# real-space/tfQMRgpu

Hardware: AMD Instinct MI355X
Metric: tfQMR solve throughput to 1e-9 residual (reference flop count / solve time); iterations/s and BSR multiply GB/s + TFLOP/s in extra keys (higher is better)
Workload: dtype f64; 1 GPU; generate_FD_example 16 120 4 2 -0.25 n 0 4 (16x16 complex<double>); mb=3573, nnzbA=17589, nnzbX_per_gpu=138229, block_columns_per_gpu=49, rhs_per_gpu=784, pairs=679189

## Files before the change

### tfqmrgpu_amd/csrc/tfq_api.hip

```cpp
#include <cstdio>
#include <cstdlib>
#include <cstring>
#include <cmath>
#include <algorithm>
#include <new>
#include <vector>
#include <dlfcn.h>

#include "tfq_device.hpp"
#include "tfq_order.hpp"
#include "tfq_vec.hpp"
#include "tfq_switch.hpp"

using namespace tfq;

namespace tfq {

static inline char lower(char c) { return char(c | 32); }

DevPlan resolve(Plan const& p) {
    DevPlan d{};
    char* b = p.buffer;
    auto at = [&](Window const& w) { return (void*)(b + w.offset); };
    d.LM = p.LM; d.LN = p.LN; d.dbl = ('z' == p.precision);
// ... 218 lines not shown
                (void)hipHostFree(p.ring); p.ring = nullptr;
                return TFQ_ERR(TFQMRGPU_STATUS_ALLOCATION_FAILED);
            }
            e = (void*)ev_;
        }
    }
    Ctl* const ring = (Ctl*)p.ring;
    hipEvent_t ev[DEPTH];
    for (int i = 0; i < DEPTH; ++i) ev[i] = (hipEvent_t)p.ringEvent[i];
    int const prof = p.profiling;
    auto const timed = [prof](int k) { return 1 == prof || (2 == prof && (TFQMRGPU_PROF_SPMM_V4_DOT == k || TFQMRGPU_PROF_SPMM_V5_NRM_DOT == k)); };
    EventList pev;
    if (prof && !pev.create(size_t(DEPTH) * (NK + 1))) return TFQ_ERR(TFQMRGPU_STATUS_ALLOCATION_FAILED);

    { RoctxRange const range(roctx(), "tfQMR preparation"); TFQ_HIP(vec_launch(VEC_SETUP, d, tol, maxIt, s), TFQMRGPU_STATUS_LAUNCH_FAILED) }
    RoctxRange const range(roctx(), "tfQMR iterations");

    tfqmrgpuStatus_t fail = TFQMRGPU_STATUS_SUCCESS;

    auto const userOp = (tfqmrgpuOperator_t)p.opFn;
    double userFlops = 0;
    size_t const vecBytes = size_t(p.nnzbX) * 2 * p.LM * p.LN * (d.dbl ? 8 : 4);
    auto const up256 = [](size_t n) { return (n + 255) & ~size_t(255); };
    if (userOp && !p.opScratch) {
        size_t const bytes = 2 * up256(vecBytes) + up256(size_t(p.nnzbX) * 4) + up256(size_t(p.nnzbX) * 2);
        TFQ_HIP(hipMalloc((void**)&p.opScratch, bytes ? bytes : 256), TFQMRGPU_STATUS_ALLOCATION_FAILED)
        char* const q = p.opScratch + 2 * up256(vecBytes);
        std::vector<uint16_t> cu(p.nnzbX);
        for (uint32_t u = 0; u < p.nnzbX; ++u) cu[u] = p.colindx[u];
        TFQ_HIP(hipMemcpyAsync(q, p.i2u.data(), size_t(p.nnzbX) * 4, hipMemcpyHostToDevice, s), TFQMRGPU_STATUS_LAUNCH_FAILED)
        TFQ_HIP(hipMemcpyAsync(q + up256(size_t(p.nnzbX) * 4), cu.data(), size_t(p.nnzbX) * 2, hipMemcpyHostToDevice, s), TFQMRGPU_STATUS_LAUNCH_FAILED)
        TFQ_HIP(hipStreamSynchronize(s), TFQMRGPU_STATUS_LAUNCH_FAILED)
    }
    auto multiply = [&](int epi, DevPlan const& d) {
        if (!userOp) { spmm_launch(epi, d, s); return; }
        char* const xu = p.opScratch; char* const yu = xu + up256(vecBytes);
        auto const i2u = (uint32_t const*)(yu + up256(vecBytes));
        auto const colU = (uint16_t const*)((char const*)i2u + up256(size_t(p.nnzbX) * 4));
        launch_convert(1, d.dbl, d.dbl, (EPI_RESIDUAL == epi) ? d.x : d.v6, xu, d.u2i, 0, p.nnzbX, p.LM, p.LN,
                       TFQMRGPU_LAYOUT_RRRRIIII, false, false, p.ilv, s);
        double fl = 0;
        auto const st = userOp(p.opCtx, yu, xu, colU, p.nnzbX, p.nCols, p.LM, p.LN, p.precision, (tfqmrgpuStream_t)s, &fl);
        if (st && !fail) fail = st;
        userFlops += fl;
        epilogue_launch(epi, d, yu, i2u, s);
    };

    static double const kOne = 1.;
    auto reduce = [&](int what) {
        if (fail && hipSuccess != hipMemcpyAsync(&d.ctl->red[3 * what + 2], &kOne, sizeof kOne, hipMemcpyHostToDevice, s)) return;
        auto const st = reduce_over_ranks(h, &d.ctl->red[3 * what], 3, s);
        if (st && !fail) fail = st;
    };
    auto launches = [&](int slot, int part, bool firstIteration) {
        DevPlan const dSlot = [&] { DevPlan x = d; x.first = firstIteration ? 1 : 0; return x; }();
        auto mark = [&](int k) {
            if (!(k < NK && timed(k)) && !(k > 0 && timed(k - 1))) return;
            if (hipSuccess != hipEventRecord(pev[slot * (NK + 1) + k], s) && !fail) fail = TFQ_ERR(TFQMRGPU_STATUS_LAUNCH_FAILED);
        };
        if (part != 2) {
            mark(TFQMRGPU_PROF_DEC35);            (void)vec_launch(VEC_DEC35, d, 0, 0, s);
            mark(TFQMRGPU_PROF_XPAY_V6);          (void)vec_launch(VEC_XPAY_V6, dSlot, 0, 0, s);
            mark(TFQMRGPU_PROF_SPMM_V4_DOT);      multiply(EPI_XPAY_DOT, dSlot);
            mark(TFQMRGPU_PROF_DEC34);            if (!fold) (void)vec_launch(VEC_DEC34, d, 0, 0, s);
            mark(TFQMRGPU_PROF_V5_NRM);           (void)vec_launch(VEC_V5_NRM, dSlot, 0, 0, s);
            mark(TFQMRGPU_PROF_DECT_C67);         if (!fold) (void)vec_launch(VEC_DECT_C67, d, 0, 0, s);
            mark(TFQMRGPU_PROF_X_V6_V7);          (void)vec_launch(VEC_X_V6_V7, dSlot, 0, 0, s);
            mark(TFQMRGPU_PROF_SPMM_V5_NRM_DOT);  multiply(EPI_AXPY_NRM_DOT, dSlot);
            mark(TFQMRGPU_PROF_DECT_FINAL);       if (!fold) (void)vec_launch(VEC_DECT_FIN, d, 0, 0, s);
            mark(TFQMRGPU_PROF_DECIDE);
            if (multi) {
                launch_decide(d, 1, s);
                reduce(0);
                launch_decide(d, 2, s);
            } else if (!fold) launch_decide(d, 0, s);
            mark(TFQMRGPU_PROF_PROBE);
        }
        if (part != 1) {
            (void)vec_launch(VEC_X_FLUSH, d, 0, 0, s);
            multiply(EPI_RESIDUAL, dSlot);
            if (!fold) (void)vec_launch(VEC_PROBE_COL, d, 0, 0, s);
            if (multi) {
                launch_probe_decide(d, 1, s);
                reduce(1);
                launch_probe_decide(d, 2, s);
            } else if (!fold) launch_probe_decide(d, 0, s);
        }
        mark(NK);
    };
    auto enqueue = [&](int slot, int part, bool firstIteration) {
        launches(slot, part, firstIteration);
        if ((hipSuccess != hipMemcpyAsync(&ring[slot], d.ctl, sizeof(Ctl), hipMemcpyDeviceToHost, s) ||
             hipSuccess != hipEventRecord(ev[slot], s)) && !fail) fail = TFQ_ERR(TFQMRGPU_STATUS_LAUNCH_FAILED);
    };

    Ctl last{};
    last.state = (maxIt > 0) ? 0 : 3; last.residual2_reached = 1e300; last.iterations_needed = maxIt;
    int enq = 0, seen = 0;
    if (userOp) {
        for (int it = 0; it < maxIt && !fail && 0 == last.state; ++it) {
            for (int part = 1; part <= 2 && !fail; ++part) {
                if (2 == part && !(0 == last.state && last.probe)) break;
                enqueue(0, part, 0 == it);
                if (hipSuccess != hipEventSynchronize(ev[0])) { fail = TFQ_ERR(TFQMRGPU_STATUS_LAUNCH_FAILED); break; }
                last = ring[0];
                if (1 == part) p.boundHistory.push_back(last.max_bound2 * histScale);
            }
            if (prof) for (int k = 0; k < NK; ++k) {
                float ms = 0;
                if (timed(k) && hipSuccess == hipEventElapsedTime(&ms, pev[k], pev[k + 1])) {
                    p.profMs[k] += ms; p.profLaunches[k] += 1;
                    if (0 == it) { p.profFirstMs[k] += ms; p.profFirstLaunches[k] += 1; }
                }
            }
        }
    } else
    while (enq < std::min(ahead, maxIt)) { enqueue(enq % DEPTH, 0, 0 == enq); ++enq; }
    while (seen < enq && (!fail || multi)) {
        int const slot = seen % DEPTH;
        if (hipSuccess != hipEventSynchronize(ev[slot])) { if (!fail) fail = TFQ_ERR(TFQMRGPU_STATUS_LAUNCH_FAILED); break; }
        int const nprobes_before = last.nprobes;
        last = ring[slot];
        ++seen;
        p.boundHistory.push_back(last.max_bound2 * histScale);
        if (prof) for (int k = 0; k < NK; ++k) {
            if (!timed(k)) continue;
            bool const gated = (TFQMRGPU_PROF_PROBE == k && last.nprobes == nprobes_before);
            float ms = 0;
            if (hipSuccess == hipEventElapsedTime(&ms, pev[slot * (NK + 1) + k], pev[slot * (NK + 1) + k + 1])) {
                if (gated) { p.profGatedMs[k] += ms; p.profGatedLaunches[k] += 1; }
                else {
                    p.profMs[k] += ms; p.profLaunches[k] += 1;
                    if (1 == seen) { p.profFirstMs[k] += ms; p.profFirstLaunches[k] += 1; }
                }
            }
        }
        if (last.state != 0) break;
        if (enq < maxIt) { enqueue(enq % DEPTH, 0, false); ++enq; }
    }
// ... 731 lines not shown
```

### tfqmrgpu_amd/csrc/tfq_colops.hpp

```cpp
#pragma once
#include "tfq_device.hpp"

namespace tfq {

#define TFQ_EPS 2.5e-308

struct ColScratch { double s[512]; double rec[2][64]; double s0[256], s1[256]; int last; };

__device__ inline void co_store(double* p, double v) { double const old = __hip_atomic_exchange(p, v, __ATOMIC_RELAXED, __HIP_MEMORY_SCOPE_AGENT); asm volatile("" :: "v"(old)); }
__device__ inline double co_load(double const* p) { return __hip_atomic_load(p, __ATOMIC_RELAXED, __HIP_MEMORY_SCOPE_AGENT); }
__device__ inline void st_record(double* p, double v, bool coherent) { if (coherent) co_store(p, v); else *p = v; }

template <int LN, int NPL, bool COH = false>
__device__ inline void column_sum(double const* part, uint32_t c0, uint32_t c1, double* s, double (&res)[NPL]) {
    constexpr int G = 256 / LN;
    constexpr int U = 16;
    int const t = threadIdx.x, g = t / LN, j = t % LN;
    double acc[NPL] = {};
    if (g < G) {
        for (uint32_t c = c0 + g; c < c1; c += U * G) {
            double v[U][NPL];
#pragma unroll
            for (int u = 0; u < U; ++u)
#pragma unroll
                for (int p = 0; p < NPL; ++p) v[u][p] = (c + u * G < c1) ? (COH ? co_load(part + (size_t(c + u * G) * NPL + p) * LN + j) : part[(size_t(c + u * G) * NPL + p) * LN + j]) : 0.;
#pragma unroll
            for (int u = 0; u < U; ++u)
                if (c + u * G < c1)
#pragma unroll
                    for (int p = 0; p < NPL; ++p) acc[p] += v[u][p];
        }
    }
    __syncthreads();
    if (g < G)
#pragma unroll
        for (int p = 0; p < NPL; ++p) s[(g * NPL + p) * LN + j] = acc[p];
    __syncthreads();
#pragma unroll
    for (int p = 0; p < NPL; ++p) res[p] = 0;
    if (t < LN) for (int gg = 0; gg < G; ++gg)
#pragma unroll
        for (int p = 0; p < NPL; ++p) res[p] += s[(gg * NPL + p) * LN + t];
}

__device__ inline bool fold_arrive(uint32_t* counter, uint32_t expected, int* lastFlag) {
    asm volatile("s_waitcnt vmcnt(0)" ::: "memory");
    __syncthreads();
    if (0 == threadIdx.x) {
        uint32_t const before = __hip_atomic_fetch_add(counter, 1u, __ATOMIC_RELAXED, __HIP_MEMORY_SCOPE_AGENT);
        int const last = (before + 1 == expected) ? 1 : 0;
        if (last) __hip_atomic_store(counter, 0u, __ATOMIC_RELAXED, __HIP_MEMORY_SCOPE_AGENT);
        *lastFlag = last;
    }
    __syncthreads();
    return *lastFlag != 0;
}

__device__ inline size_t col_part_slot(uint32_t c0, uint32_t col, uint32_t seg) { return size_t(c0 / kColSlot) + col + seg; }

template <int LN, int NPL>
__device__ inline bool column_total(DevPlan const& d, double const* part, uint32_t col, int seg, double* s, int* lastFlag, double (&res)[NPL]) {
    uint32_t const c0 = d.colChunkPtr[col], c1 = d.colChunkPtr[col + 1], n = c1 - c0;
    uint32_t const S = (seg < 0) ? 1u : col_segments(n, LN);
    if (uint32_t(seg < 0 ? 0 : seg) >= S) return false;
    if (1 == S) { if (seg < 0) column_sum<LN, NPL, true>(part, c0, c1, s, res); else column_sum<LN, NPL>(part, c0, c1, s, res); return true; }
    uint32_t const len = (n + S - 1) / S, b0 = c0 + uint32_t(seg) * len, b1 = min(c1, b0 + len);
    column_sum<LN, NPL>(part, b0, b1, s, res);
    int const t = threadIdx.x;
    if (t < LN)
#pragma unroll
        for (int p = 0; p < NPL; ++p) co_store(d.colPart + (col_part_slot(c0, col, uint32_t(seg)) * 3 + p) * LN + t, res[p]);
    if (t < 64) asm volatile("s_waitcnt vmcnt(0)" ::: "memory");
    if (0 == t) {
        uint32_t const before = __hip_atomic_fetch_add(d.foldCount + col, 1u, __ATOMIC_RELAXED, __HIP_MEMORY_SCOPE_AGENT);
        int const last = (before + 1 == S) ? 1 : 0;
        if (last) __hip_atomic_store(d.foldCount + col, 0u, __ATOMIC_RELAXED, __HIP_MEMORY_SCOPE_AGENT);
        *lastFlag = last;
    }
    __syncthreads();
    if (0 == *lastFlag) return false;
    if (t < LN) {
#pragma unroll
        for (int p = 0; p < NPL; ++p) res[p] = 0;
        constexpr int U = 8;
        for (uint32_t g0 = 0; g0 < S; g0 += U) {
            double v[U][NPL];
#pragma unroll
            for (int u = 0; u < U; ++u)
#pragma unroll
                for (int p = 0; p < NPL; ++p)
                    v[u][p] = (g0 + u < S) ? co_load(d.colPart + (col_part_slot(c0, col, g0 + u) * 3 + p) * LN + t) : 0.;
#pragma unroll
            for (int u = 0; u < U; ++u)
                if (g0 + u < S)
#pragma unroll
                    for (int p = 0; p < NPL; ++p) res[p] += v[u][p];
        }
    }
    return true;
}

template <typename R, int LN>
__device__ inline void col_dec35(DevPlan const& d, uint32_t const col, double* s, int seg, int* lastFlag) {
    int const j = threadIdx.x, jc = (j < LN) ? j : LN - 1;
    size_t const ir = (size_t(col) * 2 + 0) * LN + jc, ii = ir + LN;
    R* rho = (R*)d.rho; R* bet = (R*)d.beta;
    double const rr = double(rho[ir]), ri = double(rho[ii]);
    double z[2];
    if (!column_total<LN, 2>(d, d.pz, col, seg, s, lastFlag, z)) return;
    if (j >= LN) return;
    double const abs2rho = rr * rr + ri * ri, abs2z = z[0] * z[0] + z[1] * z[1];
    d.z[ir] = z[0]; d.z[ii] = z[1];
    if (abs2z < TFQ_EPS || abs2rho < TFQ_EPS) {
        d.status[size_t(col) * LN + j] = -1;
        bet[ir] = 0; bet[ii] = 0; rho[ir] = 0; rho[ii] = 0;
    } else {
        double const den = 1. / abs2rho;
        bet[ir] = R((z[0] * rr + z[1] * ri) * den);
        bet[ii] = R((z[1] * rr - z[0] * ri) * den);
        rho[ir] = R(z[0]); rho[ii] = R(z[1]);
    }
}

template <typename R, int LN>
__device__ inline void col_dec34(DevPlan const& d, uint32_t const col, double* s, int seg, int* lastFlag) {
    int const j = threadIdx.x, jc = (j < LN) ? j : LN - 1;
    size_t const ir = (size_t(col) * 2 + 0) * LN + jc, ii = ir + LN;
    R const* rho = (R const*)d.rho; R const* eta = (R const*)d.eta2; R* alf = (R*)d.alfa; R* c67 = (R*)d.c67a;
    double const rr = double(rho[ir]), ri = double(rho[ii]);
    double const er = double(eta[ir]), ei = double(eta[ii]), var0 = d.var[size_t(col) * LN + jc];
    double z[2];
    if (!column_total<LN, 2>(d, d.pz, col, seg, s, lastFlag, z)) return;
    if (j >= LN) return;
    double const abs2rho = rr * rr + ri * ri, abs2z = z[0] * z[0] + z[1] * z[1];
    d.z[ir] = z[0]; d.z[ii] = z[1];
    if (abs2z < TFQ_EPS || abs2rho < TFQ_EPS) {
        d.status[size_t(col) * LN + j] = -2;
        alf[ir] = 0; alf[ii] = 0; c67[ir] = 0; c67[ii] = 0;
    } else {
        double const zden = -1. / abs2z;
        alf[ir] = R((rr * z[0] + ri * z[1]) * zden);
        alf[ii] = R((ri * z[0] - rr * z[1]) * zden);
        double const vden = var0 / abs2rho;
        double const tr = (er * rr + ei * ri) * vden, ti = (ei * rr - er * ri) * vden;
        c67[ir] = R(z[0] * tr - z[1] * ti);
        c67[ii] = R(z[1] * tr + z[0] * ti);
    }
}

template <typename R, int LN, bool SETC67, bool FINAL>
__device__ inline void col_decT(DevPlan const& d, uint32_t const col, double* s, double (*rec)[64], int seg, int* lastFlag) {
    int const j = threadIdx.x, jc = (j < LN) ? j : LN - 1;
    double const Tau0 = d.tau[size_t(col) * LN + jc];
    int8_t const st0 = d.status[size_t(col) * LN + jc];
    R const alr0 = ((R const*)d.alfa)[(size_t(col) * 2 + 0) * LN + jc], ali0 = ((R const*)d.alfa)[(size_t(col) * 2 + 1) * LN + jc];
    double const invB0 = FINAL ? d.invBn2[size_t(col) * LN + jc] : 0.;
    double dd[1];
    if (!column_total<LN, 1>(d, d.pd, col, seg, s, lastFlag, dd)) return;
    if (j < LN) {
        size_t const ir = (size_t(col) * 2 + 0) * LN + j, ii = ir + LN, i1 = size_t(col) * LN + j;
        R* eta = (R*)(FINAL ? d.eta2 : d.eta); R* c67 = (R*)d.c67;
        double cosi = 0; R r67 = 1;
        double const Tau = Tau0;
        int8_t st = st0;
        double newTau;
        if (fabs(Tau) > TFQ_EPS) {
            double const Var = dd[0] / Tau;
            cosi = 1. / (1. + Var);
            d.var[i1] = Var;
            newTau = dd[0] * cosi;
            r67 = R(Var * cosi);
        } else {
            st = -3; d.status[i1] = -3;
            d.var[i1] = 0; newTau = 0;
        }
        d.tau[i1] = newTau;
        d.d[i1] = dd[0];
        if (st < 0) { eta[ir] = 0; eta[ii] = 0; }
        else { eta[ir] = R(-cosi * alr0); eta[ii] = R(-cosi * ali0); }
        if (SETC67) { c67[ir] = r67; c67[ii] = 0; }
        if (FINAL) { rec[0][j] = newTau * invB0; rec[1][j] = (st == -1 || st == -2) ? 0. : 1.; }
    }
    if (FINAL) {
        __syncthreads();
        if (0 == j) {
            double mx = 0, alive = 0;
            for (int jj = 0; jj < LN; ++jj) { if (rec[0][jj] > mx) mx = rec[0][jj]; if (rec[1][jj] > alive) alive = rec[1][jj]; }
            st_record(d.colrec + size_t(col) * 2 + 0, mx, seg < 0); st_record(d.colrec + size_t(col) * 2 + 1, alive, seg < 0);
        }
    }
}

template <int LN>
__device__ inline void col_probe(DevPlan const& d, uint32_t const col, double* s, double (*rec)[64], int seg, int* lastFlag) {
    double dd[1];
    if (!column_total<LN, 1>(d, d.pd, col, seg, s, lastFlag, dd)) return;
    int const j = threadIdx.x;
    if (j < LN) {
        size_t const i1 = size_t(col) * LN + j;
        double const res2 = dd[0] * d.invBn2[i1];
        double const tol2 = d.ctl->tol2;
        double open = 0;
        if (res2 > tol2) { if (0 == d.status[i1]) open = 1; }
        else if (res2 <= 0) d.status[i1] = 1;
        rec[0][j] = res2; rec[1][j] = open;
    }
    __syncthreads();
    if (0 == j) {
        double mx = 0, open = 0;
        for (int jj = 0; jj < LN; ++jj) { if (rec[0][jj] > mx) mx = rec[0][jj]; if (rec[1][jj] > open) open = rec[1][jj]; }
        st_record(d.colrec + size_t(col) * 2 + 0, mx, seg < 0); st_record(d.colrec + size_t(col) * 2 + 1, open, seg < 0);
    }
}

__device__ inline void decide_body(DevPlan const& d, int what, int phase, double* s0, double* s1, bool coherent = false) {
    Ctl* c = d.ctl;
    int const t = threadIdx.x;
    if (phase != 2) {
        double a = 0, b = 0;
        for (uint32_t col = t; col < d.nCols; col += 256) {
            double const u = coherent ? co_load(d.colrec + size_t(col) * 2) : d.colrec[size_t(col) * 2], v = coherent ? co_load(d.colrec + size_t(col) * 2 + 1) : d.colrec[size_t(col) * 2 + 1];
            if (u > a) a = u; if (v > b) b = v;
        }
        s0[t] = a; s1[t] = b;
        __syncthreads();
        for (int h = 128; h > 0; h >>= 1) {
            if (t < h) { if (s0[t + h] > s0[t]) s0[t] = s0[t + h]; if (s1[t + h] > s1[t]) s1[t] = s1[t + h]; }
            __syncthreads();
        }
        if (0 == t) { c->red[3 * what] = s0[0]; c->red[3 * what + 1] = s1[0]; }
        __syncthreads();
    }
    if (phase == 1 || t != 0) return;
    if (c->red[3 * what + 2] > 0.) { c->state = 4; c->probe = 0; return; }
    if (0 == what) {
        int const it = ++c->iteration;
        double const bound2 = c->red[0] * (2 * it + 1);
        c->max_bound2 = bound2;
        int probe = (bound2 <= c->target_bound2) || (it >= c->maxIterations);
        if (c->red[1] == 0.) { c->state = 2; probe = 0; }
        c->probe = probe;
        c->xpend = 1;
    } else {
        double max_res2 = 1.4e-76;
        if (c->red[3] > max_res2) max_res2 = c->red[3];
        c->target_bound2 = (c->max_bound2 / max_res2) * c->tol2;
        c->nprobes += 1;
        c->probe = 0;
        c->xpend = 0;
        double const before = c->residual2_reached;
        double const promised = (c->probe_bound2 > 0.) ? c->max_bound2 / c->probe_bound2 : 0.;
        c->residual2_reached = max_res2;
        c->probe_bound2 = c->max_bound2;
        if (c->red[4] == 0.) { c->iterations_needed = c->iteration; c->state = 1; }
        else if (c->iteration >= c->maxIterations) c->state = 3;
        else if (c->stallStop && (max_res2 > 0.49 * before || (promised > 0. && max_res2 > 9. * promised * before && max_res2 > 0.01 * before))) c->state = 3;
    }
}


enum { FOLD_DEC34 = 1, FOLD_DECT_C67 = 2, FOLD_DECT_FINAL = 3, FOLD_PROBE = 4 };

template <typename R, int LN, int WHAT>
__device__ inline void fold_tail(DevPlan const& d, uint32_t col, ColScratch& sc) {
// ... 14 lines not shown
```

### tfqmrgpu_amd/csrc/tfq_vec.hip

```cpp
#include <type_traits>

#include "tfq_device.hpp"
#include "tfq_vec.hpp"
#include "tfq_colops.hpp"

namespace tfq {


template <typename R> struct Vec;
template <> struct Vec<double> { static constexpr int N = 2; using T = double2; };
template <> struct Vec<float>  { static constexpr int N = 4; using T = float4;  };

template <int LN, int VEC> constexpr int activeThreads() {
    int t = 256;
    while (t % LN) --t;
    return t;
}

template <typename R, int LM, int LN>
struct Geo {
    static constexpr int VEC = Vec<R>::N;
    static constexpr int P = LM * LN;
    static constexpr int IPB = P / VEC;
    static constexpr int T = activeThreads<LN, VEC>();
// ... 185 lines not shown
    if (d.fold) {
        __shared__ ColScratch sc;
        fold_tail<R, LN, FOLD_DECT_C67>(d, col, sc);
    }
}

template <typename R, int LM, int LN>
__global__ __launch_bounds__(256) void k_x_v6_v7(DevPlan d) {
    using G = Geo<R, LM, LN>;
    TFQ_CHUNK_PROLOGUE(G)
    if (t >= G::T) return;
    bool const pend = (d.ctl->xpend != 0);
    R* x = (R*)d.x; R* v6 = (R*)d.v6; R* v7 = (R*)d.v7; R const* v4 = (R const*)d.v4;
    Scal<R, LN, G::VEC> eta, eta2, alfa, c67, c67a;
    eta.load((R const*)d.eta, col, t, d.ilv); eta2.load((R const*)d.eta2, col, t, d.ilv); alfa.load((R const*)d.alfa, col, t, d.ilv);
    c67.load((R const*)d.c67, col, t, d.ilv); c67a.load((R const*)d.c67a, col, t, d.ilv);
    auto sweep = [&](auto first) __attribute__((always_inline)) {
        auto item_off = [&](uint32_t w, size_t& re, size_t& im) __attribute__((always_inline)) {
            uint32_t const blk = w / G::IPB;
            re = base + size_t(blk) * 2 * G::P + size_t(w - blk * G::IPB) * G::VEC; im = re + G::P;
        };
        for (uint32_t w0 = t; w0 < nItems; w0 += 2 * G::T) {
            R sr[2][G::VEC], si[2][G::VEC], xr[2][G::VEC], xi[2][G::VEC], ar[2][G::VEC], ai[2][G::VEC], br[2][G::VEC], bi[2][G::VEC];
            size_t re[2], im[2];
            bool const two = (w0 + G::T < nItems);
            item_off(w0, re[0], im[0]); item_off(two ? w0 + G::T : w0, re[1], im[1]);
#pragma unroll
            for (int u = 0; u < 2; ++u) {
                if (u == 1 && !two) break;
                if constexpr (decltype(first)::value) {
#pragma unroll
                    for (int v = 0; v < G::VEC; ++v) { sr[u][v] = 0; si[u][v] = 0; xr[u][v] = 0; xi[u][v] = 0; }
                } else { ldv(sr[u], v7 + re[u]); ldv(si[u], v7 + im[u]); ldv(xr[u], x + re[u]); ldv(xi[u], x + im[u]); }
                ldv(ar[u], v4 + re[u]); ldv(ai[u], v4 + im[u]); ldv(br[u], v6 + re[u]); ldv(bi[u], v6 + im[u]);
            }
#pragma unroll
            for (int u = 0; u < 2; ++u) {
                if (u == 1 && !two) break;
#pragma unroll
                for (int v = 0; v < G::VEC; ++v) {
                    if (pend) axpy(xr[u][v], xi[u][v], sr[u][v], si[u][v], eta2.re[v], eta2.im[v]);
                    xpay(sr[u][v], si[u][v], br[u][v], bi[u][v], c67a.re[v], c67a.im[v]);
                    axpy(xr[u][v], xi[u][v], sr[u][v], si[u][v], eta.re[v], eta.im[v]);
                    axpy(br[u][v], bi[u][v], ar[u][v], ai[u][v], alfa.re[v], alfa.im[v]);
                    xpay(sr[u][v], si[u][v], br[u][v], bi[u][v], c67.re[v], c67.im[v]);
                }
                stv(x + re[u], xr[u]); stv(x + im[u], xi[u]); stv(v6 + re[u], br[u]); stv(v6 + im[u], bi[u]); stv(v7 + re[u], sr[u]); stv(v7 + im[u], si[u]);
            }
        }
    };
    if (d.first) sweep(std::true_type{}); else sweep(std::false_type{});
}

template <typename R, int LM, int LN>
__global__ __launch_bounds__(256) void k_x_flush(DevPlan d) {
    using G = Geo<R, LM, LN>;
    if (d.ctl->probe == 0 || d.ctl->xpend == 0) return;
    TFQ_CHUNK_PROLOGUE(G)
    if (t >= G::T) return;
    R* x = (R*)d.x; R const* v7 = (R const*)d.v7;
    Scal<R, LN, G::VEC> eta; eta.load((R const*)d.eta2, col, t, d.ilv);
    for (uint32_t w = t; w < nItems; w += G::T) {
        TFQ_ITEM_OFFSETS(G)
        R sr[G::VEC], si[G::VEC], xr[G::VEC], xi[G::VEC];
        ldv(sr, v7 + re); ldv(si, v7 + im); ldv(xr, x + re); ldv(xi, x + im);
#pragma unroll
        for (int v = 0; v < G::VEC; ++v) axpy(xr[v], xi[v], sr[v], si[v], eta.re[v], eta.im[v]);
        stv(x + re, xr); stv(x + im, xi);
    }
}

template <typename R, int LN>
__global__ __launch_bounds__(256) void k_dec35(DevPlan d) {
    if (d.ctl->state != 0) return;
    __shared__ double s[512];
    __shared__ int last;
    col_dec35<R, LN>(d, blockIdx.x, s, int(blockIdx.y), &last);
}
template <typename R, int LN>
__global__ __launch_bounds__(256) void k_dec34(DevPlan d) {
    if (d.ctl->state != 0) return;
    __shared__ double s[512];
    __shared__ int last;
    col_dec34<R, LN>(d, blockIdx.x, s, int(blockIdx.y), &last);
}
template <typename R, int LN, bool SETC67, bool FINAL>
__global__ __launch_bounds__(256) void k_decT(DevPlan d) {
    if (d.ctl->state != 0) return;
    __shared__ double s[512];
    __shared__ double rec[2][64];
    __shared__ int last;
    col_decT<R, LN, SETC67, FINAL>(d, blockIdx.x, s, rec, int(blockIdx.y), &last);
}
template <int LN>
__global__ __launch_bounds__(256) void k_probe_col(DevPlan d) {
    if (d.ctl->state != 0 || d.ctl->probe == 0) return;
    __shared__ double s[512];
    __shared__ double rec[2][64];
    __shared__ int last;
    col_probe<LN>(d, blockIdx.x, s, rec, int(blockIdx.y), &last);
}
__global__ __launch_bounds__(256) void k_decide(DevPlan d, int what, int phase) {
    if (d.ctl->state != 0) return;
    if (1 == what && 0 == d.ctl->probe) return;
    __shared__ double s0[256], s1[256];
    decide_body(d, what, phase, s0, s1);
}

template <typename R, int LM, int LN>
__global__ __launch_bounds__(256) void k_init_col(DevPlan d, double tol, int maxIterations) {
    constexpr int P = LM * LN;
    __shared__ double s[256];
    uint32_t const col = blockIdx.x;
    int const t = threadIdx.x;
    constexpr int G = 256 / LN;
    int const g = t / LN, j = t % LN;
    double acc = 0;
    if (g < G) for (uint32_t q = d.bColPtr[col]; q < d.bColPtr[col + 1]; ++q) {
        R const* b = (R const*)d.B + size_t(d.bList[q]) * 2 * P;
        for (int i = g; i < LM; i += G) {
            int const e = plane_offset(d.ilv, i, j, LN);
            double const r = b[e], im = b[P + e];
            acc = __builtin_fma(im, im, __builtin_fma(r, r, acc));
        }
    }
    if (g < G) s[g * LN + j] = acc;
    __syncthreads();
    if (t < LN) {
        double n2 = 0;
        for (int gg = 0; gg < G; ++gg) n2 += s[gg * LN + t];
        size_t const ir = (size_t(col) * 2 + 0) * LN + t, ii = ir + LN, i1 = size_t(col) * LN + t;
        d.tau[i1] = n2; d.invBn2[i1] = 1. / n2; d.var[i1] = 0; d.d[i1] = 0; d.status[i1] = 0;
        ((R*)d.rho)[ir] = 1; ((R*)d.rho)[ii] = 0;
        ((R*)d.alfa)[ir] = 0; ((R*)d.alfa)[ii] = 0; ((R*)d.beta)[ir] = 0; ((R*)d.beta)[ii] = 0;
        ((R*)d.c67)[ir] = 0; ((R*)d.c67)[ii] = 0; ((R*)d.eta)[ir] = 0; ((R*)d.eta)[ii] = 0;
        ((R*)d.c67a)[ir] = 0; ((R*)d.c67a)[ii] = 0; ((R*)d.eta2)[ir] = 0; ((R*)d.eta2)[ii] = 0;
    }
    if (0 == t) {
        d.foldCount[col] = 0;
        if (0 == col) d.foldCount[d.nCols] = 0;
    }
    if (0 == col && 0 == t) {
        Ctl* c = d.ctl;
        double const tol2 = tol * tol;
        c->tol2 = tol2; c->target_bound2 = tol2 * 100 * 100; c->max_bound2 = 0; c->residual2_reached = 1e300; c->probe_bound2 = 0;
        for (int i = 0; i < 6; ++i) c->red[i] = 0;
        c->iteration = 0; c->maxIterations = maxIterations;
        c->state = (maxIterations > 0) ? 0 : 3;
        c->probe = 0; c->iterations_needed = maxIterations; c->nprobes = 0; c->xpend = 0; c->stallStop = 0;
    }
}


// ... 142 lines not shown
    int const t = threadIdx.x;
    double u = 0, v = 0;
    for (uint32_t col = t; col < a.d.nCols; col += 256) {
        double const x = a.d.colrec[size_t(col) * 2], y = a.d.colrec[size_t(col) * 2 + 1];
        if (x > u) u = x; if (y > v) v = y;
    }
    s0[t] = u; s1[t] = v;
    __syncthreads();
    for (int h = 128; h > 0; h >>= 1) {
        if (t < h) { if (s0[t + h] > s0[t]) s0[t] = s0[t + h]; if (s1[t + h] > s1[t]) s1[t] = s1[t + h]; }
        __syncthreads();
    }
    if (0 == t) { a.refine[0] = s0[0]; a.refine[1] = s1[0]; a.refine[2] = 0; }
}

template <int LM, int LN>
__global__ __launch_bounds__(256) void k_refine_update(RefineArgs a) {
    constexpr int P = LM * LN;
    DevPlan const& d = a.d;
    uint32_t const chunk = blockIdx.x;
    uint32_t const first = d.chunkFirst[chunk], last = d.chunkFirst[chunk + 1];
    float const* const xc = (float const*)d.x;
    for (uint32_t w = threadIdx.x; w < (last - first) * 2 * P; w += 256) {
        uint32_t const blk = first + w / (2 * P);
        int const e = int(w % (2 * P)), c = e / P, r = (e % P) / LN, q = e % LN;
        double* const xz = a.xz + size_t(blk) * 2 * P + size_t(c) * P + plane_offset(a.ilvZ, r, q, LN);
        double const dx = double(xc[size_t(blk) * 2 * P + size_t(c) * P + plane_offset(d.ilv, r, q, LN)]);
        *xz = (a.cycle > 0) ? *xz + dx : dx;
    }
}

#define TFQ_SIZES(X, R) \
    X(R, 4, 4) X(R, 4, 5) X(R, 4, 8) X(R, 4, 32) X(R, 8, 8) X(R, 8, 9) X(R, 8, 10) X(R, 8, 32) X(R, 8, 64) \
    X(R, 16, 16) X(R, 16, 32) X(R, 16, 64) X(R, 32, 32) X(R, 32, 64) X(R, 64, 64)

template <typename R, int LM, int LN>
static hipError_t vec_run(int op, DevPlan const& d, double tol, int maxIt, hipStream_t s) {
    dim3 const grid(d.nChunks), cols(d.nCols, d.colSegMax ? d.colSegMax : 1), cols1(d.nCols), blk(256);
    switch (op) {
    case VEC_SETUP: {
        size_t const S = size_t(d.nnzbX) * 2 * LM * LN * sizeof(R);
        if (maxIt <= 0) if (auto const e = hipMemsetAsync(d.x, 0, S, s)) return e;
        if (!d.R) k_init_col<R, LM, LN><<<cols1, blk, 0, s>>>(d, tol, maxIt);
        k_dot35<R, LM, LN><<<grid, blk, 0, s>>>(d);
    } break;
    case VEC_DEC35:    k_dec35<R, LN><<<cols, blk, 0, s>>>(d); break;
    case VEC_XPAY_V6:  k_xpay_v6<R, LM, LN><<<grid, blk, 0, s>>>(d); break;
    case VEC_DEC34:    k_dec34<R, LN><<<cols, blk, 0, s>>>(d); break;
    case VEC_V5_NRM:   k_v5_nrm<R, LM, LN><<<grid, blk, 0, s>>>(d); break;
    case VEC_DECT_C67: k_decT<R, LN, true, false><<<cols, blk, 0, s>>>(d); break;
    case VEC_X_V6_V7:  k_x_v6_v7<R, LM, LN><<<grid, blk, 0, s>>>(d); break;
    case VEC_DECT_FIN: k_decT<R, LN, false, true><<<cols, blk, 0, s>>>(d); break;
    case VEC_X_FLUSH:  k_x_flush<R, LM, LN><<<grid, blk, 0, s>>>(d); break;
    case VEC_PROBE_COL: k_probe_col<LN><<<cols, blk, 0, s>>>(d); break;
    }
    return hipSuccess;
}

hipError_t vec_launch(int op, DevPlan const& d, double tol, int maxIt, hipStream_t s) {
    int const key = d.LM * 1000 + d.LN;
#define TFQ_CASE(R, LM, LN) case LM * 1000 + LN: return vec_run<R, LM, LN>(op, d, tol, maxIt, s);
    if (d.dbl) { switch (key) { TFQ_SIZES(TFQ_CASE, double) default: break; } }
    else       { switch (key) { TFQ_SIZES(TFQ_CASE, float)  default: break; } }
#undef TFQ_CASE
    return hipErrorInvalidValue;
}

template <int LM, int LN>
static void refine_run(int what, RefineArgs const& a, hipStream_t s) {
    dim3 const grid(a.d.nChunks), cols(a.d.nCols), blk(256);
    bool const quads = (4 == a.d.ilv) && (0 == a.ilvZ || 2 == a.ilvZ);
    if (0 == what) {
        if constexpr (LM % 4 == 0) {
            if (quads && 2 == a.ilvZ) k_refine_residual_q<LM, LN, 2><<<grid, blk, 0, s>>>(a);
            else if (quads) k_refine_residual_q<LM, LN, 0><<<grid, blk, 0, s>>>(a);
            else k_refine_residual<LM, LN><<<grid, blk, 0, s>>>(a);
        } else k_refine_residual<LM, LN><<<grid, blk, 0, s>>>(a);
        k_refine_init_col<LN><<<cols, blk, 0, s>>>(a);
        k_refine_max<<<1, blk, 0, s>>>(a);
    } else {
        if constexpr (LM % 4 == 0) {
            if (quads && 2 == a.ilvZ) k_refine_update_q<LM, LN, 2><<<grid, blk, 0, s>>>(a);
            else if (quads) k_refine_update_q<LM, LN, 0><<<grid, blk, 0, s>>>(a);
            else k_refine_update<LM, LN><<<grid, blk, 0, s>>>(a);
        } else k_refine_update<LM, LN><<<grid, blk, 0, s>>>(a);
    }
}
static void refine_dispatch(int what, RefineArgs const& a, hipStream_t s) {
    int const key = a.d.LM * 1000 + a.d.LN;
#define TFQ_CASE(R, LM, LN) case LM * 1000 + LN: refine_run<LM, LN>(what, a, s); break;
    switch (key) { TFQ_SIZES(TFQ_CASE, float) default: break; }
#undef TFQ_CASE
}
void launch_refine_residual(RefineArgs const& a, hipStream_t s) { refine_dispatch(0, a, s); }
void launch_refine_update(RefineArgs const& a, hipStream_t s)   { refine_dispatch(1, a, s); }

void launch_decide(DevPlan const& d, int phase, hipStream_t s)       { k_decide<<<1, 256, 0, s>>>(d, 0, phase); }
void launch_probe_decide(DevPlan const& d, int phase, hipStream_t s) { k_decide<<<1, 256, 0, s>>>(d, 1, phase); }

}
```

### tfqmrgpu_amd/csrc/tfq_vec.hpp

```cpp
#pragma once
#include "tfq_device.hpp"

namespace tfq {

enum {
    VEC_SETUP = 0,
    VEC_DEC35,
    VEC_XPAY_V6,
    VEC_DEC34,
    VEC_V5_NRM,
    VEC_DECT_C67,
    VEC_X_V6_V7,
    VEC_DECT_FIN,
    VEC_X_FLUSH,
    VEC_PROBE_COL
};

hipError_t vec_launch(int op, DevPlan const& d, double tol, int maxIt, hipStream_t s);

void spmm_launch(int epi, DevPlan const& d, hipStream_t s);

char const* spmm_kernel_family(DevPlan const& d);

void spmm_apply(DevPlan const& d, void const* X, void* Y, hipStream_t s);

void epilogue_launch(int epi, DevPlan const& d, void const* Yext, uint32_t const* i2u, hipStream_t s);

}
```

Before: 20.91 TFLOP/s.

## Fuse final decT with next dec35 and decide into one column kernel

Adds a join mode, on by default when fold is off, that merges the final tau/eta column reduction and the next iteration's rho/beta (dec35) reduction into one kernel. It reads pd and pz together through a generic record accessor. A last-block-arrives counter then runs the convergence decision inside that kernel, and the probe column kernel does the same. The x flush kernel becomes grid-strided with a capped grid and skips work when the state is no longer running. The aim is fewer small launches and fewer passes over the partial sums per iteration, in exchange for atomic coordination and the first dec35 being handled separately.

```diff
diff --git a/tfqmrgpu_amd/csrc/tfq_api.hip b/tfqmrgpu_amd/csrc/tfq_api.hip
--- a/tfqmrgpu_amd/csrc/tfq_api.hip
+++ b/tfqmrgpu_amd/csrc/tfq_api.hip
@@ -294,6 +294,8 @@
         auto const st = reduce_over_ranks(h, &d.ctl->red[3 * what], 3, s);
         if (st && !fail) fail = st;
     };
+    static int const joinEnv = lab_switch("TFQMRGPU_JOIN", 1);
+    bool const join = (0 != joinEnv) && !fold;
     auto launches = [&](int slot, int part, bool firstIteration) {
         DevPlan const dSlot = [&] { DevPlan x = d; x.first = firstIteration ? 1 : 0; return x; }();
         auto mark = [&](int k) {
@@ -301,7 +303,7 @@
             if (hipSuccess != hipEventRecord(pev[slot * (NK + 1) + k], s) && !fail) fail = TFQ_ERR(TFQMRGPU_STATUS_LAUNCH_FAILED);
         };
         if (part != 2) {
-            mark(TFQMRGPU_PROF_DEC35);            (void)vec_launch(VEC_DEC35, d, 0, 0, s);
+            mark(TFQMRGPU_PROF_DEC35);            if (!join || firstIteration) (void)vec_launch(VEC_DEC35, d, 0, 0, s);
             mark(TFQMRGPU_PROF_XPAY_V6);          (void)vec_launch(VEC_XPAY_V6, dSlot, 0, 0, s);
             mark(TFQMRGPU_PROF_SPMM_V4_DOT);      multiply(EPI_XPAY_DOT, dSlot);
             mark(TFQMRGPU_PROF_DEC34);            if (!fold) (void)vec_launch(VEC_DEC34, d, 0, 0, s);
@@ -309,24 +311,25 @@
             mark(TFQMRGPU_PROF_DECT_C67);         if (!fold) (void)vec_launch(VEC_DECT_C67, d, 0, 0, s);
             mark(TFQMRGPU_PROF_X_V6_V7);          (void)vec_launch(VEC_X_V6_V7, dSlot, 0, 0, s);
             mark(TFQMRGPU_PROF_SPMM_V5_NRM_DOT);  multiply(EPI_AXPY_NRM_DOT, dSlot);
-            mark(TFQMRGPU_PROF_DECT_FINAL);       if (!fold) (void)vec_launch(VEC_DECT_FIN, d, 0, 0, s);
+            mark(TFQMRGPU_PROF_DECT_FINAL);       if (join) (void)vec_launch(multi ? VEC_FIN35 : VEC_FIN35_DECIDE, d, 0, 0, s);
+                                                  else if (!fold) (void)vec_launch(VEC_DECT_FIN, d, 0, 0, s);
             mark(TFQMRGPU_PROF_DECIDE);
             if (multi) {
                 launch_decide(d, 1, s);
                 reduce(0);
                 launch_decide(d, 2, s);
-            } else if (!fold) launch_decide(d, 0, s);
+            } else if (!fold && !join) launch_decide(d, 0, s);
             mark(TFQMRGPU_PROF_PROBE);
         }
         if (part != 1) {
-            (void)vec_launch(VEC_X_FLUSH, d, 0, 0, s);
+            (void)vec_launch(join ? VEC_X_FLUSH_STRIDED : VEC_X_FLUSH, d, 0, 0, s);
             multiply(EPI_RESIDUAL, dSlot);
-            if (!fold) (void)vec_launch(VEC_PROBE_COL, d, 0, 0, s);
+            if (!fold) (void)vec_launch((join && !multi) ? VEC_PROBE_COL_DECIDE : VEC_PROBE_COL, d, 0, 0, s);
             if (multi) {
                 launch_probe_decide(d, 1, s);
                 reduce(1);
                 launch_probe_decide(d, 2, s);
-            } else if (!fold) launch_probe_decide(d, 0, s);
+            } else if (!fold && !join) launch_probe_decide(d, 0, s);
         }
         mark(NK);
     };
diff --git a/tfqmrgpu_amd/csrc/tfq_colops.hpp b/tfqmrgpu_amd/csrc/tfq_colops.hpp
--- a/tfqmrgpu_amd/csrc/tfq_colops.hpp
+++ b/tfqmrgpu_amd/csrc/tfq_colops.hpp
@@ -4,6 +4,8 @@
 namespace tfq {
 
 #define TFQ_EPS 2.5e-308
+
+__device__ inline void decide_body(DevPlan const& d, int what, int phase, double* s0, double* s1, bool coherent);
 
 struct ColScratch { double s[512]; double rec[2][64]; double s0[256], s1[256]; int last; };
 
@@ -11,8 +13,8 @@
 __device__ inline double co_load(double const* p) { return __hip_atomic_load(p, __ATOMIC_RELAXED, __HIP_MEMORY_SCOPE_AGENT); }
 __device__ inline void st_record(double* p, double v, bool coherent) { if (coherent) co_store(p, v); else *p = v; }
 
-template <int LN, int NPL, bool COH = false>
-__device__ inline void column_sum(double const* part, uint32_t c0, uint32_t c1, double* s, double (&res)[NPL]) {
+template <int LN, int NPL, typename Rec>
+__device__ inline void column_sum_of(Rec const& rec, uint32_t c0, uint32_t c1, double* s, double (&res)[NPL]) {
     constexpr int G = 256 / LN;
     constexpr int U = 16;
     int const t = threadIdx.x, g = t / LN, j = t % LN;
@@ -23,7 +25,7 @@
 #pragma unroll
             for (int u = 0; u < U; ++u)
 #pragma unroll
-                for (int p = 0; p < NPL; ++p) v[u][p] = (c + u * G < c1) ? (COH ? co_load(part + (size_t(c + u * G) * NPL + p) * LN + j) : part[(size_t(c + u * G) * NPL + p) * LN + j]) : 0.;
+                for (int p = 0; p < NPL; ++p) v[u][p] = (c + u * G < c1) ? rec(c + u * G, p, j) : 0.;
 #pragma unroll
             for (int u = 0; u < U; ++u)
                 if (c + u * G < c1)
@@ -41,6 +43,10 @@
     if (t < LN) for (int gg = 0; gg < G; ++gg)
 #pragma unroll
         for (int p = 0; p < NPL; ++p) res[p] += s[(gg * NPL + p) * LN + t];
+}
+template <int LN, int NPL, bool COH = false>
+__device__ inline void column_sum(double const* part, uint32_t c0, uint32_t c1, double* s, double (&res)[NPL]) {
+    column_sum_of<LN, NPL>([part](uint32_t c, int p, int j) { return COH ? co_load(part + (size_t(c) * NPL + p) * LN + j) : part[(size_t(c) * NPL + p) * LN + j]; }, c0, c1, s, res);
 }
 
 __device__ inline bool fold_arrive(uint32_t* counter, uint32_t expected, int* lastFlag) {
@@ -58,14 +64,15 @@
 
 __device__ inline size_t col_part_slot(uint32_t c0, uint32_t col, uint32_t seg) { return size_t(c0 / kColSlot) + col + seg; }
 
-template <int LN, int NPL>
-__device__ inline bool column_total(DevPlan const& d, double const* part, uint32_t col, int seg, double* s, int* lastFlag, double (&res)[NPL]) {
+template <int LN, int NPL, typename Rec>
+__device__ inline bool column_total_of(DevPlan const& d, Rec const& rec, uint32_t col, int seg, double* s, int* lastFlag, double (&res)[NPL]) {
+    static_assert(NPL <= 3, "DevPlan::colPart holds three planes per slot");
     uint32_t const c0 = d.colChunkPtr[col], c1 = d.colChunkPtr[col + 1], n = c1 - c0;
-    uint32_t const S = (seg < 0) ? 1u : col_segments(n, LN);
-    if (uint32_t(seg < 0 ? 0 : seg) >= S) return false;
-    if (1 == S) { if (seg < 0) column_sum<LN, NPL, true>(part, c0, c1, s, res); else column_sum<LN, NPL>(part, c0, c1, s, res); return true; }
+    uint32_t const S = col_segments(n, LN);
+    if (uint32_t(seg) >= S) return false;
+    if (1 == S) { column_sum_of<LN, NPL>(rec, c0, c1, s, res); return true; }
     uint32_t const len = (n + S - 1) / S, b0 = c0 + uint32_t(seg) * len, b1 = min(c1, b0 + len);
-    column_sum<LN, NPL>(part, b0, b1, s, res);
+    column_sum_of<LN, NPL>(rec, b0, b1, s, res);
     int const t = threadIdx.x;
     if (t < LN)
 #pragma unroll
@@ -99,20 +106,23 @@
     }
     return true;
 }
-
-template <typename R, int LN>
-__device__ inline void col_dec35(DevPlan const& d, uint32_t const col, double* s, int seg, int* lastFlag) {
-    int const j = threadIdx.x, jc = (j < LN) ? j : LN - 1;
-    size_t const ir = (size_t(col) * 2 + 0) * LN + jc, ii = ir + LN;
+template <int LN, int NPL>
+__device__ inline bool column_total(DevPlan const& d, double const* part, uint32_t col, int seg, double* s, int* lastFlag, double (&res)[NPL]) {
+    if (seg < 0) {
+        column_sum<LN, NPL, true>(part, d.colChunkPtr[col], d.colChunkPtr[col + 1], s, res);
+        return true;
+    }
+    return column_total_of<LN, NPL>(d, [part](uint32_t c, int p, int j) { return part[(size_t(c) * NPL + p) * LN + j]; }, col, seg, s, lastFlag, res);
+}
+
+template <typename R, int LN, bool MARK = true>
+__device__ inline void dec35_update(DevPlan const& d, uint32_t const col, int j, double const (&z)[2], double rr, double ri) {
+    size_t const ir = (size_t(col) * 2 + 0) * LN + j, ii = ir + LN;
     R* rho = (R*)d.rho; R* bet = (R*)d.beta;
-    double const rr = double(rho[ir]), ri = double(rho[ii]);
-    double z[2];
-    if (!column_total<LN, 2>(d, d.pz, col, seg, s, lastFlag, z)) return;
-    if (j >= LN) return;
     double const abs2rho = rr * rr + ri * ri, abs2z = z[0] * z[0] + z[1] * z[1];
     d.z[ir] = z[0]; d.z[ii] = z[1];
     if (abs2z < TFQ_EPS || abs2rho < TFQ_EPS) {
-        d.status[size_t(col) * LN + j] = -1;
+        if (MARK) d.status[size_t(col) * LN + j] = -1;
         bet[ir] = 0; bet[ii] = 0; rho[ir] = 0; rho[ii] = 0;
     } else {
         double const den = 1. / abs2rho;
@@ -120,6 +130,17 @@
         bet[ii] = R((z[1] * rr - z[0] * ri) * den);
         rho[ir] = R(z[0]); rho[ii] = R(z[1]);
     }
+}
+template <typename R, int LN>
+__device__ inline void col_dec35(DevPlan const& d, uint32_t const col, double* s, int seg, int* lastFlag) {
+    int const j = threadIdx.x, jc = (j < LN) ? j : LN - 1;
+    size_t const ir = (size_t(col) * 2 + 0) * LN + jc, ii = ir + LN;
+    R const* rho = (R const*)d.rho;
+    double const rr = double(rho[ir]), ri = double(rho[ii]);
+    double z[2];
+    if (!column_total<LN, 2>(d, d.pz, col, seg, s, lastFlag, z)) return;
+    if (j >= LN) return;
+    dec35_update<R, LN>(d, col, j, z, rr, ri);
 }
 
 template <typename R, int LN>
@@ -148,15 +169,21 @@
     }
 }
 
+template <typename R>
+struct DecTIn { double Tau0, invB0; R alr0, ali0; int8_t st0; };
+template <typename R, int LN, bool FINAL>
+__device__ inline DecTIn<R> decT_fetch(DevPlan const& d, uint32_t const col, int jc) {
+    DecTIn<R> in;
+    in.Tau0 = d.tau[size_t(col) * LN + jc];
+    in.st0 = d.status[size_t(col) * LN + jc];
+    in.alr0 = ((R const*)d.alfa)[(size_t(col) * 2 + 0) * LN + jc]; in.ali0 = ((R const*)d.alfa)[(size_t(col) * 2 + 1) * LN + jc];
+    in.invB0 = FINAL ? d.invBn2[size_t(col) * LN + jc] : 0.;
+    return in;
+}
 template <typename R, int LN, bool SETC67, bool FINAL>
-__device__ inline void col_decT(DevPlan const& d, uint32_t const col, double* s, double (*rec)[64], int seg, int* lastFlag) {
-    int const j = threadIdx.x, jc = (j < LN) ? j : LN - 1;
-    double const Tau0 = d.tau[size_t(col) * LN + jc];
-    int8_t const st0 = d.status[size_t(col) * LN + jc];
-    R const alr0 = ((R const*)d.alfa)[(size_t(col) * 2 + 0) * LN + jc], ali0 = ((R const*)d.alfa)[(size_t(col) * 2 + 1) * LN + jc];
-    double const invB0 = FINAL ? d.invBn2[size_t(col) * LN + jc] : 0.;
-    double dd[1];
-    if (!column_total<LN, 1>(d, d.pd, col, seg, s, lastFlag, dd)) return;
+__device__ inline void decT_update(DevPlan const& d, uint32_t const col, DecTIn<R> const& in, double const (&dd)[1], double (*rec)[64], bool coherent) {
+    int const j = threadIdx.x;
+    double const Tau0 = in.Tau0, invB0 = in.invB0; R const alr0 = in.alr0, ali0 = in.ali0; int8_t const st0 = in.st0;
     if (j < LN) {
         size_t const ir = (size_t(col) * 2 + 0) * LN + j, ii = ir + LN, i1 = size_t(col) * LN + j;
         R* eta = (R*)(FINAL ? d.eta2 : d.eta); R* c67 = (R*)d.c67;
@@ -186,12 +213,39 @@
         if (0 == j) {
             double mx = 0, alive = 0;
             for (int jj = 0; jj < LN; ++jj) { if (rec[0][jj] > mx) mx = rec[0][jj]; if (rec[1][jj] > alive) alive = rec[1][jj]; }
-            st_record(d.colrec + size_t(col) * 2 + 0, mx, seg < 0); st_record(d.colrec + size_t(col) * 2 + 1, alive, seg < 0);
-        }
-    }
-}
-
-template <int LN>
+            st_record(d.colrec + size_t(col) * 2 + 0, mx, coherent); st_record(d.colrec + size_t(col) * 2 + 1, alive, coherent);
+        }
+    }
+}
+template <typename R, int LN, bool SETC67, bool FINAL>
+__device__ inline void col_decT(DevPlan const& d, uint32_t const col, double* s, double (*rec)[64], int seg, int* lastFlag) {
+    int const j = threadIdx.x, jc = (j < LN) ? j : LN - 1;
+    DecTIn<R> const in = decT_fetch<R, LN, FINAL>(d, col, jc);
+    double dd[1];
+    if (!column_total<LN, 1>(d, d.pd, col, seg, s, lastFlag, dd)) return;
+    decT_update<R, LN, SETC67, FINAL>(d, col, in, dd, rec, seg < 0);
+}
+
+template <typename R, int LN, bool DECIDE>
+__device__ inline void col_fin35(DevPlan const& d, uint32_t const col, double* s, double (*rec)[64], int seg, int* lastFlag) {
+    int const j = threadIdx.x, jc = (j < LN) ? j : LN - 1;
+    DecTIn<R> const in = decT_fetch<R, LN, true>(d, col, jc);
+    R const* rho = (R const*)d.rho;
+    double const rr = double(rho[(size_t(col) * 2 + 0) * LN + jc]), ri = double(rho[(size_t(col) * 2 + 1) * LN + jc]);
+    double const* const pd = d.pd; double const* const pz = d.pz;
+    double t3[3];
+    if (!column_total_of<LN, 3>(d, [pd, pz](uint32_t c, int p, int jj) { return (0 == p) ? pd[size_t(c) * LN + jj] : pz[(size_t(c) * 2 + (p - 1)) * LN + jj]; },
+                                col, seg, s, lastFlag, t3)) return;
+    double const dd[1] = { t3[0] }, z[2] = { t3[1], t3[2] };
+    decT_update<R, LN, false, true>(d, col, in, dd, rec, DECIDE);
+    if (j < LN) dec35_update<R, LN, false>(d, col, j, z, rr, ri);
+    if (DECIDE) {
+        if (!fold_arrive(d.foldCount + d.nCols, d.nCols, lastFlag)) return;
+        decide_body(d, 0, 0, s, s + 256, true);
+    }
+}
+
+template <int LN, bool DECIDE = false>
 __device__ inline void col_probe(DevPlan const& d, uint32_t const col, double* s, double (*rec)[64], int seg, int* lastFlag) {
     double dd[1];
     if (!column_total<LN, 1>(d, d.pd, col, seg, s, lastFlag, dd)) return;
@@ -209,7 +263,11 @@
     if (0 == j) {
         double mx = 0, open = 0;
         for (int jj = 0; jj < LN; ++jj) { if (rec[0][jj] > mx) mx = rec[0][jj]; if (rec[1][jj] > open) open = rec[1][jj]; }
-        st_record(d.colrec + size_t(col) * 2 + 0, mx, seg < 0); st_record(d.colrec + size_t(col) * 2 + 1, open, seg < 0);
+        st_record(d.colrec + size_t(col) * 2 + 0, mx, DECIDE || seg < 0); st_record(d.colrec + size_t(col) * 2 + 1, open, DECIDE || seg < 0);
+    }
+    if (DECIDE) {
+        if (!fold_arrive(d.foldCount + d.nCols, d.nCols, lastFlag)) return;
+        decide_body(d, 1, 0, s, s + 256, true);
     }
 }
 
diff --git a/tfqmrgpu_amd/csrc/tfq_vec.hip b/tfqmrgpu_amd/csrc/tfq_vec.hip
--- a/tfqmrgpu_amd/csrc/tfq_vec.hip
+++ b/tfqmrgpu_amd/csrc/tfq_vec.hip
@@ -261,21 +261,27 @@
     if (d.first) sweep(std::true_type{}); else sweep(std::false_type{});
 }
 
+constexpr uint32_t kFlushGrid = 256 * 8;
 template <typename R, int LM, int LN>
 __global__ __launch_bounds__(256) void k_x_flush(DevPlan d) {
     using G = Geo<R, LM, LN>;
-    if (d.ctl->probe == 0 || d.ctl->xpend == 0) return;
-    TFQ_CHUNK_PROLOGUE(G)
+    if (d.ctl->state != 0 || d.ctl->probe == 0 || d.ctl->xpend == 0) return;
+    int const t = threadIdx.x;
     if (t >= G::T) return;
     R* x = (R*)d.x; R const* v7 = (R const*)d.v7;
-    Scal<R, LN, G::VEC> eta; eta.load((R const*)d.eta2, col, t, d.ilv);
-    for (uint32_t w = t; w < nItems; w += G::T) {
-        TFQ_ITEM_OFFSETS(G)
-        R sr[G::VEC], si[G::VEC], xr[G::VEC], xi[G::VEC];
-        ldv(sr, v7 + re); ldv(si, v7 + im); ldv(xr, x + re); ldv(xi, x + im);
-#pragma unroll
-        for (int v = 0; v < G::VEC; ++v) axpy(xr[v], xi[v], sr[v], si[v], eta.re[v], eta.im[v]);
-        stv(x + re, xr); stv(x + im, xi);
+    for (uint32_t chunk = blockIdx.x; chunk < d.nChunks; chunk += gridDim.x) {
+        uint32_t const first = d.chunkFirst[chunk];
+        uint32_t const nItems = (d.chunkFirst[chunk + 1] - first) * G::IPB;
+        size_t const base = size_t(first) * 2 * G::P;
+        Scal<R, LN, G::VEC> eta; eta.load((R const*)d.eta2, d.chunkCol[chunk], t, d.ilv);
+        for (uint32_t w = t; w < nItems; w += G::T) {
+            TFQ_ITEM_OFFSETS(G)
+            R sr[G::VEC], si[G::VEC], xr[G::VEC], xi[G::VEC];
+            ldv(sr, v7 + re); ldv(si, v7 + im); ldv(xr, x + re); ldv(xi, x + im);
+#pragma unroll
+            for (int v = 0; v < G::VEC; ++v) axpy(xr[v], xi[v], sr[v], si[v], eta.re[v], eta.im[v]);
+            stv(x + re, xr); stv(x + im, xi);
+        }
     }
 }
 
@@ -308,6 +314,22 @@
     __shared__ double rec[2][64];
     __shared__ int last;
     col_probe<LN>(d, blockIdx.x, s, rec, int(blockIdx.y), &last);
+}
+template <typename R, int LN, bool DECIDE>
+__global__ __launch_bounds__(256) void k_fin35(DevPlan d) {
+    if (d.ctl->state != 0) return;
+    __shared__ double s[768];
+    __shared__ double rec[2][64];
+    __shared__ int last;
+    col_fin35<R, LN, DECIDE>(d, blockIdx.x, s, rec, int(blockIdx.y), &last);
+}
+template <int LN>
+__global__ __launch_bounds__(256) void k_probe_col_decide(DevPlan d) {
+    if (d.ctl->state != 0 || d.ctl->probe == 0) return;
+    __shared__ double s[512];
+    __shared__ double rec[2][64];
+    __shared__ int last;
+    col_probe<LN, true>(d, blockIdx.x, s, rec, int(blockIdx.y), &last);
 }
 __global__ __launch_bounds__(256) void k_decide(DevPlan d, int what, int phase) {
     if (d.ctl->state != 0) return;
@@ -556,7 +578,11 @@
     case VEC_X_V6_V7:  k_x_v6_v7<R, LM, LN><<<grid, blk, 0, s>>>(d); break;
     case VEC_DECT_FIN: k_decT<R, LN, false, true><<<cols, blk, 0, s>>>(d); break;
     case VEC_X_FLUSH:  k_x_flush<R, LM, LN><<<grid, blk, 0, s>>>(d); break;
+    case VEC_X_FLUSH_STRIDED: k_x_flush<R, LM, LN><<<dim3(d.nChunks < kFlushGrid ? d.nChunks : kFlushGrid), blk, 0, s>>>(d); break;
     case VEC_PROBE_COL: k_probe_col<LN><<<cols, blk, 0, s>>>(d); break;
+    case VEC_FIN35:        k_fin35<R, LN, false><<<cols, blk, 0, s>>>(d); break;
+    case VEC_FIN35_DECIDE: k_fin35<R, LN, true><<<cols, blk, 0, s>>>(d); break;
+    case VEC_PROBE_COL_DECIDE: k_probe_col_decide<LN><<<cols, blk, 0, s>>>(d); break;
     }
     return hipSuccess;
 }
diff --git a/tfqmrgpu_amd/csrc/tfq_vec.hpp b/tfqmrgpu_amd/csrc/tfq_vec.hpp
--- a/tfqmrgpu_amd/csrc/tfq_vec.hpp
+++ b/tfqmrgpu_amd/csrc/tfq_vec.hpp
@@ -13,7 +13,11 @@
     VEC_X_V6_V7,
     VEC_DECT_FIN,
     VEC_X_FLUSH,
-    VEC_PROBE_COL
+    VEC_PROBE_COL,
+    VEC_FIN35,
+    VEC_FIN35_DECIDE,
+    VEC_PROBE_COL_DECIDE,
+    VEC_X_FLUSH_STRIDED
 };
 
 hipError_t vec_launch(int op, DevPlan const& d, double tol, int maxIt, hipStream_t s);
```

Result: no change. 20.99 TFLOP/s, median of 6 (+0.4%).
